# bayesian-optimization/BayesianOptimization

Measured on AMD Instinct MI355X. Metric: acquisition candidates/sec (suggest step: GP fit at fixed theta + posterior + acquisition + arg-best), higher is better.
Workload: dtype f64

## Files before the change

### bayesianoptimization_amd/csrc/posterior_kernel_v2.hip

```cpp
#include <type_traits>

#include "gpbo_internal.h"
#include "fit_bodies.h"
#include "i8_digits.h"
#include "posterior_tile.h"

namespace gpbo {

typedef double d4 __attribute__((ext_vector_type(4)));

constexpr int V2_CANDS = 64;
constexpr int V2_STRIDE = 64;

struct PostArgs2 {
  const double* Wp;
  const double* Xs;
  const double* alpha;
  const double* Xcs;
  double* part;
  double* mu_part;
  PostGrid g;
  const double* Kst;
  int64_t ldk;
  int64_t m0;
// ... 138 lines not shown

  __syncthreads();
  {
    double kv0[E];
    gen_compute(0, kv0, 1.0);
    gen_store(kv0, 0);
  }
  double2 aA[2], aB[2];
  loadA(0, aA);
  __syncthreads();

  const int last_stage = n_stages - 1;
  const int last_pair = (int)pairs - 1;
  auto stage = [&](int st, auto mode) {
    constexpr int MODE = decltype(mode)::value;
    const int buf = st & 1;
    double kv[E];
    if constexpr (MODE > 0) loadA(min(KP * st + 1, last_pair), aB);
    gen_compute(min(st + 1, last_stage), kv, st < last_stage ? 1.0 : 0.0);
    if constexpr (GEN == 2) __builtin_amdgcn_sched_barrier(0);
    if constexpr (MODE > 0) {
#pragma unroll
      for (int pp = 0; pp < KP; ++pp) {
        if (pp & 1) mma_pair(buf, pp, aB, mode);
        else mma_pair(buf, pp, aA, mode);
        if (pp + 1 < KP || (pp & 1) == 0) {
          if (pp & 1) loadA(min(KP * st + pp + 2, last_pair), aB);
          else loadA(min(KP * st + pp + 2, last_pair), aA);
        }
      }
    }
    gen_store(kv, buf ^ 1);
    __syncthreads();
  };
  const int sA = min(last_stage, (rowA0 + 15) / BK);
  const int sB = min(last_stage, (rowB0 + 15) / BK);
  int s = 0;
  for (; s <= sA; ++s) stage(s, both_t{});
  for (; s <= sB; ++s) stage(s, later_t{});
  for (; s <= last_stage; ++s) stage(s, std::integral_constant<int, 0>{});

  static_assert(2 * WAVES * V2_CANDS <= 2 * BK * V2_STRIDE, "the epilogue's exchange area aliases the stage tiles");
  double* red = Ks;
  double* mured = Ks + WAVES * V2_CANDS;
#pragma unroll
  for (int jt = 0; jt < 4; ++jt) {
    double v = 0.0;
#pragma unroll
    for (int rr = 0; rr < 4; ++rr) v = fma(acc[0][jt][rr], acc[0][jt][rr], v);
    if (!activeA) v = 0.0;
    double vb = 0.0;
#pragma unroll
    for (int rr = 0; rr < 4; ++rr) vb = fma(acc[1][jt][rr], acc[1][jt][rr], vb);
    if (activeB) v += vb;
    v += __shfl_xor(v, 16);
    v += __shfl_xor(v, 32);
    if (lane < 16) red[wave * V2_CANDS + jt * 16 + lane] = v;
  }
  mured[wave * V2_CANDS + lane] = mu_acc;
  __syncthreads();
  if (tid < V2_CANDS) {
    double v = 0.0;
#pragma unroll
    for (int w = 0; w < WAVES; ++w) v += red[w * V2_CANDS + tid];
    const int64_t m = p.m0 + (int64_t)ct * V2_CANDS + tid;
    if (GEN != 2 && p.fuse_ends) {
      double u = 0.0;
#pragma unroll
      for (int w = 0; w < WAVES; ++w) u += mured[w * V2_CANDS + tid];
      if (m < p.ends.M)
        posterior_finalize_elem(0.0 + v, 0.0 + u, p.ends.y_mean, p.ends.y_std, p.ends.amplitude, p.ends.white, p.ends.mu + m, p.ends.sd + m, p.ends.negvar);
      return;
    }
    p.part[(int64_t)r * p.g.Mp + m] = v;
    if (GEN != 2 && last) {
      double u = 0.0;
#pragma unroll
      for (int w = 0; w < WAVES; ++w) u += mured[w * V2_CANDS + tid];
      p.mu_part[m] = u;
    }
  }
}

constexpr int GEN_CH = 64;
template <PostPath SLAB> struct slab_value { using type = double; };
template <> struct slab_value<PostPath::SlabF32> { using type = float; };
template <int DP, int KERNEL, PostPath SLAB>
__global__ __launch_bounds__(256) void kstar_gen_kernel(const double* __restrict__ Xs, const double* __restrict__ alpha,
                                                        const double* __restrict__ Xcs, void* __restrict__ slab,
                                                        int64_t ldk, int NP, double* __restrict__ mu_part,
                                                        int64_t Mp, int64_t m0) {
  static_assert(SLAB == PostPath::SlabF64 || SLAB == PostPath::SlabF32 || SLAB == PostPath::SlabI8, "a slab path");
  __shared__ __attribute__((aligned(16))) double xs[GEN_CH * DP];
  __shared__ double al[GEN_CH];
  const int64_t ml = (int64_t)blockIdx.x * 256 + threadIdx.x;
  const bool live = ml < ldk;
  const int k0 = blockIdx.y * POST_ROWS, k1 = min(NP, k0 + POST_ROWS);
  double xc[DP];
  {
    const double* xcp = Xcs + (m0 + (live ? ml : 0)) * DP;
#pragma unroll
    for (int t = 0; t < DP; t += 2) {
      const double2 v = *reinterpret_cast<const double2*>(xcp + t);
      xc[t] = v.x;
      xc[t + 1] = v.y;
    }
  }
  double mu = 0.0;
  auto pair = [&](int kk, double& ka, double& kb) {
    const double* xr = xs + kk * DP;
    double d2a = 0.0, d2b = 0.0;
#pragma unroll
    for (int t = 0; t < DP; ++t) {
      const double da = xc[t] - xr[t], db = xc[t] - xr[DP + t];
      d2a = fma(da, da, d2a);
      d2b = fma(db, db, d2b);
    }
    ka = gpbo_kernel_value<KERNEL>(d2a);
    kb = gpbo_kernel_value<KERNEL>(d2b);
  };
  auto mean = [&](int kk, double ka, double kb) {
    mu = fma(ka, al[kk], mu);
    mu = fma(kb, al[kk + 1], mu);
  };
  for (int kc = k0; kc < k1; kc += GEN_CH) {
    __syncthreads();
    {
      const double2* src = reinterpret_cast<const double2*>(Xs + (int64_t)kc * DP);
      double2* dst = reinterpret_cast<double2*>(xs);
      for (int e = threadIdx.x; e < GEN_CH * DP / 2; e += 256) dst[e] = src[e];
      if (threadIdx.x < GEN_CH) al[threadIdx.x] = alpha[kc + threadIdx.x];
    }
    __syncthreads();
    if (!live) continue;
    if constexpr (SLAB == PostPath::SlabI8) {
      constexpr int S = I8_S;
      uint4* Kd = static_cast<uint4*>(slab);
      const int64_t cb = i8_kd_block(ml >> 4, NP);
#pragma unroll 1
      for (int kg = 0; kg < GEN_CH; kg += 16) {
        uint32_t w[S][4] = {};
#pragma unroll
        for (int kk = kg; kk < kg + 16; kk += 2) {
          double ka, kb;
          pair(kk, ka, kb);
          mean(kk, ka, kb);
          const int64_t qa = i8_quantize<S>(ka), qb = i8_quantize<S>(kb);
          const int j = kk - kg;
#pragma unroll
          for (int t = 0; t < S; ++t) {
            w[t][j >> 2] |= (uint32_t)((qa >> (8 * (S - 1 - t))) & 255) << (8 * (j & 3));
            w[t][j >> 2] |= (uint32_t)((qb >> (8 * (S - 1 - t))) & 255) << (8 * ((j + 1) & 3));
          }
        }
        const int k = kc + kg;
        uint4* dst = Kd + i8_frag_index<S>(cb, k, 0, (int)(ml & 15));
#pragma unroll
        for (int t = 0; t < S; ++t) {
          const uint32_t x = t ? 0x80808080u : 0u;
          dst[t * 64] = make_uint4(w[t][0] ^ x, w[t][1] ^ x, w[t][2] ^ x, w[t][3] ^ x);
        }
      }
    } else {
      using T = typename slab_value<SLAB>::type;
      T* Kst = static_cast<T*>(slab);
#pragma unroll 2
      for (int kk = 0; kk < GEN_CH; kk += 2) {
        double ka, kb;
        pair(kk, ka, kb);
        const int k = kc + kk;
        Kst[(int64_t)k * ldk + ml] = (T)ka;
        Kst[(int64_t)(k + 1) * ldk + ml] = (T)kb;
        mean(kk, ka, kb);
      }
    }
  }
  if (live) mu_part[(int64_t)blockIdx.y * Mp + m0 + ml] = mu;
}

template <PostPath SLAB>
static int launch_gen(gpbo_ctx* ctx, Model& m, void* slab, int64_t ldk, int64_t Mp, int64_t m0, int nchunks) {
  return with_dp_kernel(ctx, m.DP, m.kernel, [&](auto dp, auto k) {
    kstar_gen_kernel<decltype(dp)::value, decltype(k)::value, SLAB><<<dim3((unsigned)((ldk + 255) / 256), (unsigned)nchunks), dim3(256), 0,
                                                                      ctx->stream>>>(m.Xs, m.alpha, ctx->Xcs, slab, ldk, (int)m.NP,
                                                                                     ctx->mu_part, Mp, m0);
    GPBO_HIP(ctx, hipGetLastError());
    return GPBO_OK;
  });
}

int launch_kstar_slab(gpbo_ctx* ctx, Model& m, double* Kst, int64_t ldk, int64_t Mp, int64_t m0, int nchunks) {
  return launch_gen<PostPath::SlabF64>(ctx, m, Kst, ldk, Mp, m0, nchunks);
}
int launch_kstar_slab_f32(gpbo_ctx* ctx, Model& m, float* Kst, int64_t ldk, int64_t Mp, int64_t m0, int nchunks) {
  return launch_gen<PostPath::SlabF32>(ctx, m, Kst, ldk, Mp, m0, nchunks);
}
int launch_kstar_digits(gpbo_ctx* ctx, Model& m, void* Kd, int64_t ldk, int64_t Mp, int64_t m0, int nchunks) {
  return launch_gen<PostPath::SlabI8>(ctx, m, Kd, ldk, Mp, m0, nchunks);
}

static PostArgs2 post_args(gpbo_ctx* ctx, const Model& m, int64_t Mp, int nchunks, int64_t ncands) {
  PostArgs2 a;
  a.Wp = m.Wp; a.Xs = m.Xs; a.alpha = m.alpha; a.Xcs = ctx->Xcs; a.part = ctx->part; a.mu_part = ctx->mu_part;
  a.g = {(int)m.NP, Mp, nchunks, (int)(ncands / V2_CANDS)};
  a.Kst = nullptr; a.ldk = 0; a.m0 = 0;
  return a;
}

int launch_slab_gemm_f64(gpbo_ctx* ctx, Model& m, const double* slab, int64_t ldk, int64_t m0, int64_t Mp, int part_chunks) {
  PostArgs2 a = post_args(ctx, m, Mp, part_chunks, ldk);
  a.Kst = slab; a.ldk = ldk; a.m0 = m0;
  const size_t lds = (size_t)(2 * 32 * V2_STRIDE) * sizeof(double);
  posterior_kernel_v2<4, 0, 2, 32><<<dim3((unsigned)a.g.blocks()), dim3(512), lds, ctx->stream>>>(a);
  GPBO_HIP(ctx, hipGetLastError());
  return GPBO_OK;
}

int launch_posterior_fused(gpbo_ctx* ctx, Model& m, int64_t Mp, const PostPlan& plan, const PostEnds& ends) {
  if (plan.fuse_ends && plan.part_chunks != 1) GPBO_FAIL(ctx, GPBO_ERR_STATE, "posterior: fused ends need one row chunk");
  PostArgs2 a = post_args(ctx, m, Mp, plan.part_chunks, Mp);
  const int64_t nblocks = a.g.blocks();
  if (nblocks > 0x7fffffffLL) GPBO_FAIL(ctx, GPBO_ERR_UNSUPPORTED, "posterior: grid too large; shard the candidates");
  if (plan.fuse_ends) { a.fuse_ends = 1; a.ends = ends; }
  const bool wide = plan.path == PostPath::Fused512;
  return with_dp_kernel(ctx, m.DP, m.kernel, [&](auto dp, auto k) {
    constexpr int DP = decltype(dp)::value, KERNEL = decltype(k)::value;
    if (wide) {
      const size_t lds = (size_t)(2 * 32 * V2_STRIDE + DP * V2_CANDS) * sizeof(double);
      posterior_kernel_v2<DP, KERNEL, 1, 32, 16><<<dim3((unsigned)nblocks), dim3(1024), lds, ctx->stream>>>(a);
    } else {
      const size_t lds = (size_t)(2 * POST_BK * V2_STRIDE + DP * V2_CANDS) * sizeof(double);
      posterior_kernel_v2<DP, KERNEL, 1><<<dim3((unsigned)nblocks), dim3(512), lds, ctx->stream>>>(a);
    }
    GPBO_HIP(ctx, hipGetLastError());
    return GPBO_OK;
  });
}

}

#ifdef GPBO_DEBUG
using namespace gpbo;

int gpbo_debug_i8_kstar_digits(gpbo_ctx* ctx, int64_t NP, int64_t m0, int64_t ldk, void* Kd_out, double* kst_out, double* mu_part_out) {
  if (!ctx) return GPBO_ERR_INVALID;
  Model& m = ctx->models[0];
  if (!m.fitted || ctx->pending_info[0]) GPBO_FAIL(ctx, GPBO_ERR_STATE, "debug_i8_kstar_digits: model slot 0 has not been fitted");
  if (ctx->M < 1) GPBO_FAIL(ctx, GPBO_ERR_STATE, "debug_i8_kstar_digits: no candidates resident (call gpbo_set_candidates)");
  if (ctx->d_c != m.d) GPBO_FAIL(ctx, GPBO_ERR_INVALID, "debug_i8_kstar_digits: candidate dimension differs from the fitted model");
  const int64_t Mp = round_up(ctx->M, POST_CANDS);
  if (!Kd_out || !kst_out || !mu_part_out || m0 < 0 || ldk < 64 || m0 % 64 || ldk % 64 || m0 + ldk > Mp)
    GPBO_FAIL(ctx, GPBO_ERR_INVALID, "debug_i8_kstar_digits: bad arguments (m0, ldk multiples of 64 inside the padded candidate set)");
  if (m.NP > I8_NP_MAX || m.NP % 64) GPBO_FAIL(ctx, GPBO_ERR_UNSUPPORTED, "debug_i8_kstar_digits: the int8 GEMM serves NP <= 16384");
  if (NP != m.NP)
    GPBO_FAIL(ctx, GPBO_ERR_INVALID, "debug_i8_kstar_digits: NP is not the padded size of the model in slot 0");
  GPBO_HIP(ctx, hipSetDevice(ctx->device));
// ... 29 lines not shown
```

### bayesianoptimization_amd/csrc/posterior_plan.h

```cpp
#pragma once

#include <cstdint>

namespace gpbo {

constexpr int POST_ROWS = 256;
constexpr int POST_ROWS_WIDE = 512;
constexpr int POST_CANDS = 128;
constexpr int I8_ROWS = 128;
constexpr int64_t I8_NP_MIN = 2048;
constexpr int I8_NP_MAX = 16384;
constexpr int I8_S = 7;

enum class PostPath {
  Small,
  Fused256,
  Fused512,
  SlabF64,
  SlabI8,
  SlabF32,
};

struct PostPlan {
  PostPath path;
  bool fuse_ends;
  int part_chunks;
  int mu_chunks;
};

inline bool f32_use_mfma32(int64_t NP) { return NP >= POST_ROWS_WIDE; }

inline bool posterior_i8_serves(int64_t NP) { return NP >= I8_NP_MIN && NP <= I8_NP_MAX; }

struct SlabSpec {
  int64_t bytes_per_cand;
  int64_t offset_cap;
  bool narrow_ok;
};
inline SlabSpec slab_spec(PostPath path, int64_t NP) {
  switch (path) {
    case PostPath::SlabF64: return {8 * NP, (int64_t)80 * 1000 * 1000, false};
    case PostPath::SlabF32: return {4 * NP, (int64_t)160 * 1000 * 1000, false};
    case PostPath::SlabI8: return {I8_S * NP, INT64_MAX, true};
    default: return {0, 0, false};
  }
}
inline int64_t slab_doubles(int64_t ms, int64_t bytes_per_cand) { return (ms * bytes_per_cand + 7) / 8; }

constexpr int64_t I8_SLAB_BYTES = 256 * 1000 * 1000;
inline int64_t i8_slab_width(int64_t NP, int64_t bytes_per_cand, int64_t granted, int64_t compute_units) {
  const int64_t chunks = (NP + POST_ROWS - 1) / POST_ROWS;
  const int64_t kmax = I8_SLAB_BYTES / bytes_per_cand / 256;
  int64_t width = I8_SLAB_BYTES / bytes_per_cand / 128 * 128;
  int64_t best_wgs = 0, best_cap = 1;
  for (int64_t k = kmax; k >= 1 && 2 * k > kmax; --k) {
    const int64_t wgs = k * chunks, cap = (wgs + compute_units - 1) / compute_units * compute_units;
    if (wgs * best_cap > best_wgs * cap) { best_wgs = wgs; best_cap = cap; width = 256 * k; }
  }
  if (granted < width) width = granted;
  return width < 128 ? 128 : width;
}

inline PostPlan plan_posterior(int64_t NP, int64_t M, bool f32, int64_t gemv_limit, int force_kernel = 0, bool no_small = false,
                               bool no_fuse_ends = false) {
  const int nchunks = (int)((NP + POST_ROWS - 1) / POST_ROWS);
  const int64_t Mp = (M + POST_CANDS - 1) / POST_CANDS * POST_CANDS;
  if (M <= gemv_limit && !no_small) return {PostPath::Small, false, 0, 0};
  if (f32)
    return {PostPath::SlabF32, false, f32_use_mfma32(NP) ? (int)((NP + POST_ROWS_WIDE - 1) / POST_ROWS_WIDE) : nchunks, nchunks};
  PostPath path;
  if (nchunks <= 1) path = PostPath::Fused256;
  else if (nchunks == 2) {
    if (Mp < 8192) path = PostPath::Fused256;
    else if (Mp < 9216) path = PostPath::SlabF64;
    else if (Mp <= 16384) path = PostPath::Fused512;
    else if (Mp < 32768) path = PostPath::Fused256;
    else path = NP >= 384 ? PostPath::Fused512 : PostPath::SlabF64;
  } else path = posterior_i8_serves(NP) ? PostPath::SlabI8 : PostPath::SlabF64;
  switch (force_kernel) {
    case 2: path = PostPath::Fused256; break;
    case 3: path = PostPath::SlabF64; break;
    case 4: if (NP <= 1024) path = PostPath::Fused512; break;
    case 8: if (NP > 512 && NP <= I8_NP_MAX) path = PostPath::SlabI8; break;
  }
  PostPlan p{path, false, nchunks, nchunks};
  if (path == PostPath::Fused256 || path == PostPath::Fused512) {
    if (path == PostPath::Fused512) p.part_chunks = (int)((NP + POST_ROWS_WIDE - 1) / POST_ROWS_WIDE);
    p.mu_chunks = 1;
    p.fuse_ends = p.part_chunks == 1 && !no_fuse_ends;
  } else if (path == PostPath::SlabI8) {
    p.part_chunks = (int)((NP + I8_ROWS - 1) / I8_ROWS);
  }
  return p;
}

}
```

### bayesianoptimization_amd/csrc/i8_digits.h

```cpp
#pragma once

#include <cmath>
#include <cstdint>

#include "posterior_plan.h"

#if defined(__HIPCC__)
#define GPBO_HD __host__ __device__
#else
#define GPBO_HD
#endif

namespace gpbo {

static_assert((int64_t)I8_S * 128 * 128 * I8_NP_MAX < ((int64_t)1 << 31), "int32 level sums overflow at I8_NP_MAX");

template <int S>
GPBO_HD constexpr int64_t i8_offset() {
  int64_t o = 0;
  for (int t = 1; t < S; ++t) o = o * 256 + 128;
  return o;
}

GPBO_HD inline int64_t i8_round(double x) {
#if defined(__HIP_DEVICE_COMPILE__)
  return __double2ll_rn(x);
#else
  return (int64_t)std::nearbyint(x);
#endif
}

template <int S>
GPBO_HD inline int64_t i8_quantize(double x) {
  return i8_round(std::ldexp(x, 8 * S - 2)) + i8_offset<S>();
}

template <int S>
GPBO_HD inline uint32_t i8_digit_byte(int64_t Qo, int t) {
  return (uint32_t)((Qo >> (8 * (S - 1 - t))) & 255) ^ (t ? 128u : 0u);
}

GPBO_HD inline int i8_row_exponent(double maxabs) {
  int e = 0;
  (void)std::frexp(maxabs, &e);
  return maxabs > 0.0 ? e : 0;
}

template <int S>
GPBO_HD constexpr int64_t i8_frag_index(int64_t first_step, int64_t k, int plane, int item) {
  return ((first_step + (k >> 6)) * S + plane) * 64 + ((k >> 4) & 3) * 16 + item;
}
GPBO_HD constexpr int64_t i8_kd_block(int64_t cb, int64_t NP) { return cb * (NP / 64); }
GPBO_HD constexpr int64_t i8_wd_block(int64_t b) {
  const int64_t q = b >> 2, r = b & 3;
  return b + 2 * q * (q - 1) + r * q;
}

template <int S>
GPBO_HD inline double i8_combine(const int32_t* acc) {
  static_assert(S >= 5 && S <= 7, "groups of S - 4, 2 and 2 levels");
  double h = 0.0;
  for (int l = 0; l < S - 4; ++l) h = h * 256.0 + (double)acc[l];
  h *= 4294967296.0;
  const double m = (double)acc[S - 4] * 16777216.0 + (double)acc[S - 3] * 65536.0;
  const double lo = (double)acc[S - 2] * 256.0 + (double)acc[S - 1];
  const double s = h + m;
  const double bb = s - h;
  const double e = (h - (s - bb)) + (m - bb);
  return s + (e + lo);
}

template <int S>
GPBO_HD constexpr int i8_scale_exp(int e) {
  return e - 2 * (8 * S - 2) + 8 * (S - 1);
}

}
```

### bayesianoptimization_amd/csrc/posterior_i8.hip

```cpp
#include <algorithm>

#include "gpbo_internal.h"
#include "i8_digits.h"
#include "posterior_tile.h"

namespace gpbo {

typedef int v4i __attribute__((ext_vector_type(4)));

constexpr int I8_CANDS = 64;

__global__ __launch_bounds__(256) void wd_row_scale_kernel(const double* __restrict__ W, int* __restrict__ wexp,
                                                           double* __restrict__ wscale, int64_t N, int64_t NP) {
  const int64_t row = (int64_t)blockIdx.x * 4 + (threadIdx.x >> 6);
  const int lane = threadIdx.x & 63;
  if (row >= NP) return;
  double mx = 0.0;
  if (row < N)
    for (int64_t j = lane; j <= row; j += 64) mx = fmax(mx, fabs(W[row * NP + j]));
#pragma unroll
  for (int o = 32; o > 0; o >>= 1) mx = fmax(mx, __shfl_xor(mx, o));
  if (lane == 0) {
    const int e = i8_row_exponent(mx);
    wexp[row] = e;
    wscale[row] = ldexp(1.0, i8_scale_exp<I8_S>(e));
  }
}

__global__ __launch_bounds__(256) void wd_pack_kernel(const double* __restrict__ W, const int* __restrict__ wexp,
                                                      uint4* __restrict__ Wd, int64_t N, int64_t NP) {
  const int b = blockIdx.y;
  const int t = blockIdx.x * 256 + threadIdx.x;
  const int ks = t >> 6, lane = t & 63;
  if (ks > b / 4) return;
  const int64_t row = (int64_t)b * 16 + (lane & 15);
  const int64_t c0 = (int64_t)ks * 64 + (lane >> 4) * 16;
  const int e = wexp[row];
  uint32_t w[I8_S][4] = {};
#pragma unroll
  for (int j = 0; j < 16; ++j) {
    const int64_t col = c0 + j;
    const double x = (row < N && col < N && col <= row) ? W[row * NP + col] : 0.0;
    const int64_t q = i8_quantize<I8_S>(ldexp(x, -e));
#pragma unroll
    for (int s = 0; s < I8_S; ++s) w[s][j >> 2] |= i8_digit_byte<I8_S>(q, s) << (8 * (j & 3));
  }
  uint4* dst = Wd + i8_frag_index<I8_S>(i8_wd_block(b), c0, 0, lane & 15);
#pragma unroll
  for (int s = 0; s < I8_S; ++s) dst[s * 64] = make_uint4(w[s][0], w[s][1], w[s][2], w[s][3]);
}

static int pack_wd(gpbo_ctx* ctx, Model& m) {
  const int64_t nb = m.NP / 16;
  int rc;
  if ((rc = ensure(ctx, &m.Wd, &m.cap_Wd, i8_wd_block(nb) * I8_S * 64))) return rc;
  if ((rc = ensure(ctx, &m.wscale, &m.cap_wscale, 2 * m.NP))) return rc;
  int* wexp = reinterpret_cast<int*>(m.wscale + m.NP);
  wd_row_scale_kernel<<<dim3((unsigned)((m.NP + 3) / 4)), dim3(256), 0, ctx->stream>>>(m.W, wexp, m.wscale, m.N, m.NP);
  GPBO_HIP(ctx, hipGetLastError());
  wd_pack_kernel<<<dim3((unsigned)((m.NP + 255) / 256), (unsigned)nb), dim3(256), 0, ctx->stream>>>(m.W, wexp, m.Wd, m.N, m.NP);
  GPBO_HIP(ctx, hipGetLastError());
  m.wd_valid = true;
  return GPBO_OK;
}

struct I8Args {
  const uint4* Wd;
  const double* wscale;
  const uint4* Kd;
  double* part;
  PostGrid g;
  int64_t m0;
};

template <int S>
__global__ __launch_bounds__(256, 1) void posterior_i8_kernel(I8Args p) {
  const int tid = threadIdx.x;
  const int wave = __builtin_amdgcn_readfirstlane(tid >> 6);
  const int lane = tid & 63;
  int r, ct;
  p.g.map(blockIdx.x, r, ct);
  const int nks = p.g.NP / 64;
  const int rb = r * (I8_ROWS / 32) + wave;
  const bool active = rb < p.g.NP / 32;

  __shared__ double red[4][I8_CANDS];
  double ss[4] = {0.0, 0.0, 0.0, 0.0};
  if (active) {
    v4i acc[2][4][S];
#pragma unroll
    for (int a = 0; a < 2; ++a)
#pragma unroll
      for (int j = 0; j < 4; ++j)
#pragma unroll
        for (int l = 0; l < S; ++l) acc[a][j][l] = v4i{};
    const int n = rb / 2 + 1;
    const uint4* wa = p.Wd + i8_wd_block(2 * rb) * S * 64;
    const uint4* kb0 = p.Kd + i8_kd_block(4 * ct, p.g.NP) * S * 64;
    const __amdgpu_buffer_rsrc_t rsA = __builtin_amdgcn_make_buffer_rsrc(const_cast<uint4*>(wa), 0, 0x7fffffff, BUF_FLAGS);
    const __amdgpu_buffer_rsrc_t rsB = __builtin_amdgcn_make_buffer_rsrc(const_cast<uint4*>(kb0), 0, 0x7fffffff, BUF_FLAGS);
    const unsigned voff = (unsigned)lane * 16u;
    const unsigned sofA = (unsigned)n * S * 1024u, sofB = (unsigned)nks * S * 1024u;
    v4i a[2][S], b[4][S];
    auto load_a = [&](int ks, int i) {
      const unsigned o = (unsigned)ks * S * 1024u + i * sofA;
#pragma unroll
      for (int s = 0; s < S; ++s)
        a[i][s] = __builtin_bit_cast(v4i, __builtin_amdgcn_raw_buffer_load_b128(rsA, voff, o + s * 1024u, 0));
    };
    auto load_b = [&](int ks, int j0) {
      const unsigned o = (unsigned)ks * S * 1024u;
#pragma unroll
      for (int s = 0; s < S; ++s)
#pragma unroll
        for (int j = j0; j < j0 + 2; ++j)
          b[j][s] = __builtin_bit_cast(v4i, __builtin_amdgcn_raw_buffer_load_b128(rsB, voff, o + j * sofB + s * 1024u, 0));
    };
    auto mma = [&](int i, int j0) {
#pragma unroll
      for (int s = 0; s < S; ++s)
#pragma unroll
        for (int t = 0; t + s < S; ++t)
#pragma unroll
          for (int j = j0; j < j0 + 2; ++j)
            acc[i][j][s + t] = __builtin_amdgcn_mfma_i32_16x16x64_i8(a[i][s], b[j][t], acc[i][j][s + t], 0, 0, 0);
    };
    load_a(0, 0);
    load_b(0, 0);
    __builtin_amdgcn_sched_barrier(0);
    load_a(0, 1);
    __builtin_amdgcn_sched_barrier(0);
    load_b(0, 2);
#pragma unroll 1
    for (int ks = 0; ks < n; ++ks) {
      const int nx = min(ks + 1, n - 1);
      __builtin_amdgcn_sched_barrier(0);
      mma(0, 0);
      __builtin_amdgcn_sched_barrier(0);
      mma(1, 0);
      __builtin_amdgcn_sched_barrier(0);
      load_b(nx, 0);
      __builtin_amdgcn_sched_barrier(0);
      mma(0, 2);
      __builtin_amdgcn_sched_barrier(0);
      load_a(nx, 0);
      __builtin_amdgcn_sched_barrier(0);
      mma(1, 2);
      __builtin_amdgcn_sched_barrier(0);
      load_a(nx, 1);
      load_b(nx, 2);
    }

#pragma unroll
    for (int j = 0; j < 4; ++j) {
      double s = 0.0;
#pragma unroll
      for (int a = 0; a < 2; ++a) {
        double v[4];
#pragma unroll
        for (int i = 0; i < 4; ++i) {
          const int row = rb * 32 + 16 * a + 4 * (lane >> 4) + i;
          int32_t lv[S];
#pragma unroll
          for (int l = 0; l < S; ++l) lv[l] = acc[a][j][l][i];
          v[i] = i8_combine<S>(lv) * p.wscale[row];
          __builtin_amdgcn_sched_barrier(0);
        }
#pragma unroll
        for (int i = 0; i < 4; ++i) s = fma(v[i], v[i], s);
        s = __shfl_xor(s, 32);
#pragma unroll
        for (int i = 0; i < 4; ++i) s = fma(v[i], v[i], s);
        if (a == 0) s = __shfl_xor(s, 32);
      }
      ss[j] = s;
    }
  }
#pragma unroll
  for (int j = 0; j < 4; ++j) {
    const double o = __shfl_xor(ss[j], 16);
    if ((lane >> 4) == 2) red[wave][j * 16 + (lane & 15)] = ss[j] + o;
  }
  __syncthreads();
  if (tid < I8_CANDS) {
    const double v = ((red[0][tid] + red[1][tid]) + red[2][tid]) + red[3][tid];
    p.part[(int64_t)r * p.g.Mp + p.m0 + (int64_t)ct * I8_CANDS + tid] = v;
  }
}

static int launch_i8_gemm(gpbo_ctx* ctx, const uint4* Wd, const double* wscale, const uint4* Kd, double* part, int64_t NP, int64_t Mp,
                          int nchunks, int64_t ldk, int64_t m0) {
  I8Args a;
  a.Wd = Wd; a.wscale = wscale; a.Kd = Kd; a.part = part;
  a.g = {(int)NP, Mp, nchunks, (int)(ldk / I8_CANDS)};
  a.m0 = m0;
  posterior_i8_kernel<I8_S><<<dim3((unsigned)a.g.blocks()), dim3(256), 0, ctx->stream>>>(a);
  GPBO_HIP(ctx, hipGetLastError());
  return GPBO_OK;
}

int launch_slab_gemm_i8(gpbo_ctx* ctx, Model& m, const void* slab, int64_t ldk, int64_t m0, int64_t Mp, int part_chunks) {
  return launch_i8_gemm(ctx, m.Wd, m.wscale, static_cast<const uint4*>(slab), ctx->part, m.NP, Mp, part_chunks, ldk, m0);
}

int prepare_posterior_i8(gpbo_ctx* ctx, Model& m) {
  if (m.NP > I8_NP_MAX || m.NP % 64) GPBO_FAIL(ctx, GPBO_ERR_UNSUPPORTED, "posterior: the int8 GEMM serves NP <= 16384");
  int rc;
  if (!m.wd_valid && (rc = pack_wd(ctx, m))) return rc;
  if (!ctx->compute_units) GPBO_HIP(ctx, hipDeviceGetAttribute(&ctx->compute_units, hipDeviceAttributeMultiprocessorCount, ctx->device));
  return GPBO_OK;
}

}

#ifdef GPBO_DEBUG
using namespace gpbo;

static bool i8_debug_np_ok(int64_t NP) { return NP >= 64 && NP <= I8_NP_MAX && NP % 64 == 0; }

int gpbo_debug_i8_pack_w(gpbo_ctx* ctx, const double* W, int64_t N, int64_t NP, void* Wd_out, int* wexp_out, double* wscale_out) {
  if (!ctx) return GPBO_ERR_INVALID;
  if (!W || !Wd_out || !wexp_out || !wscale_out || !i8_debug_np_ok(NP) || N < 1 || N > NP)
    GPBO_FAIL(ctx, GPBO_ERR_INVALID, "debug_i8_pack_w: bad arguments (NP a multiple of 64 in [64, 16384], 1 <= N <= NP)");
  GPBO_HIP(ctx, hipSetDevice(ctx->device));
  Model m;
  m.N = N; m.NP = NP;
  auto done = [&](int code) {
    if (m.W) (void)hipFree(m.W);
    if (m.Wd) (void)hipFree(m.Wd);
    if (m.wscale) (void)hipFree(m.wscale);
    return code;
  };
  const size_t sq = (size_t)NP * NP * sizeof(double);
  if (hipMalloc((void**)&m.W, sq) != hipSuccess) return done(GPBO_ERR_HIP);
  if (hipMemcpy(m.W, W, sq, hipMemcpyHostToDevice) != hipSuccess) return done(GPBO_ERR_HIP);
  int rc = pack_wd(ctx, m);
  if (rc) return done(rc);
  if (hipStreamSynchronize(ctx->stream) != hipSuccess) return done(GPBO_ERR_HIP);
  const size_t wd_bytes = (size_t)i8_wd_block(NP / 16) * I8_S * 64 * sizeof(uint4);
  if (hipMemcpy(Wd_out, m.Wd, wd_bytes, hipMemcpyDeviceToHost) != hipSuccess) return done(GPBO_ERR_HIP);
  if (hipMemcpy(wscale_out, m.wscale, (size_t)NP * sizeof(double), hipMemcpyDeviceToHost) != hipSuccess) return done(GPBO_ERR_HIP);
  if (hipMemcpy(wexp_out, m.wscale + NP, (size_t)NP * sizeof(int), hipMemcpyDeviceToHost) != hipSuccess) return done(GPBO_ERR_HIP);
  return done(GPBO_OK);
}

int gpbo_debug_i8_gemm(gpbo_ctx* ctx, const void* Wd, const double* wscale, const void* Kd, int64_t NP, int64_t M, double* part_out) {
  if (!ctx) return GPBO_ERR_INVALID;
  if (!Wd || !wscale || !Kd || !part_out || !i8_debug_np_ok(NP) || M < I8_CANDS || M % I8_CANDS || M > (1 << 20))
    GPBO_FAIL(ctx, GPBO_ERR_INVALID, "debug_i8_gemm: bad arguments (NP a multiple of 64 in [64, 16384], M a multiple of 64)");
  GPBO_HIP(ctx, hipSetDevice(ctx->device));
  const int nchunks = (int)((NP + I8_ROWS - 1) / I8_ROWS);
  const size_t wd_bytes = (size_t)i8_wd_block(NP / 16) * I8_S * 64 * sizeof(uint4);
  const size_t kd_bytes = (size_t)M * NP * I8_S;
  const size_t part_bytes = (size_t)nchunks * M * sizeof(double);
  uint4 *dW = nullptr, *dK = nullptr;
  double *dS = nullptr, *dP = nullptr;
  auto done = [&](int code) {
    if (dW) (void)hipFree(dW);
    if (dK) (void)hipFree(dK);
    if (dS) (void)hipFree(dS);
    if (dP) (void)hipFree(dP);
    return code;
  };
  if (hipMalloc((void**)&dW, wd_bytes) != hipSuccess || hipMalloc((void**)&dK, kd_bytes) != hipSuccess ||
      hipMalloc((void**)&dS, (size_t)NP * sizeof(double)) != hipSuccess || hipMalloc((void**)&dP, part_bytes) != hipSuccess)
    return done(GPBO_ERR_HIP);
  if (hipMemcpy(dW, Wd, wd_bytes, hipMemcpyHostToDevice) != hipSuccess || hipMemcpy(dK, Kd, kd_bytes, hipMemcpyHostToDevice) != hipSuccess ||
      hipMemcpy(dS, wscale, (size_t)NP * sizeof(double), hipMemcpyHostToDevice) != hipSuccess ||
      hipMemset(dP, 0xff, part_bytes) != hipSuccess)
    return done(GPBO_ERR_HIP);
  const int rc = launch_i8_gemm(ctx, dW, dS, dK, dP, NP, M, nchunks, M, 0);
  if (rc) return done(rc);
  if (hipStreamSynchronize(ctx->stream) != hipSuccess) return done(GPBO_ERR_HIP);
  if (hipMemcpy(part_out, dP, part_bytes, hipMemcpyDeviceToHost) != hipSuccess) return done(GPBO_ERR_HIP);
  return done(GPBO_OK);
}
#endif
```

Before: 6.108 million.

## Software-pipeline LDS reads in K* slab generator with register ring and larger staging

The slab generation kernel now stages up to 32KB of training points per sync (up to POST_ROWS points instead of a fixed 64). Distance computation is split into 4-dimension pieces, prefetched from LDS into a register ring one or more pieces ahead, with sched_barrier and asm pins keeping loads overlapped with FMAs. Alpha for the next pair is also prefetched. This is meant to hide LDS latency and reduce syncthreads count, at the cost of more registers and occupancy risk.

```diff
diff --git a/bayesianoptimization_amd/csrc/posterior_kernel_v2.hip b/bayesianoptimization_amd/csrc/posterior_kernel_v2.hip
--- a/bayesianoptimization_amd/csrc/posterior_kernel_v2.hip
+++ b/bayesianoptimization_amd/csrc/posterior_kernel_v2.hip
@@ -244,7 +244,9 @@
   }
 }
 
-constexpr int GEN_CH = 64;
+#define GEN_PIN(a, b) asm volatile("" : "+v"(a), "+v"(b) : : "memory")
+constexpr int GEN_PIECE = 4;
+constexpr int gen_ring_slots(int DP) { return DP >= 64 ? 2 : DP / GEN_PIECE < 4 ? DP / GEN_PIECE : 4; }
 template <PostPath SLAB> struct slab_value { using type = double; };
 template <> struct slab_value<PostPath::SlabF32> { using type = float; };
 template <int DP, int KERNEL, PostPath SLAB>
@@ -253,8 +255,13 @@
                                                         int64_t ldk, int NP, double* __restrict__ mu_part,
                                                         int64_t Mp, int64_t m0) {
   static_assert(SLAB == PostPath::SlabF64 || SLAB == PostPath::SlabF32 || SLAB == PostPath::SlabI8, "a slab path");
-  __shared__ __attribute__((aligned(16))) double xs[GEN_CH * DP];
-  __shared__ double al[GEN_CH];
+  constexpr int PTS = gen_stage_points(DP);
+  constexpr int NPIECE = DP / GEN_PIECE;
+  constexpr int RING = gen_ring_slots(DP);
+  static_assert(DP % GEN_PIECE == 0 && NPIECE % RING == 0, "a piece's ring slot is its index modulo the ring, the same in every pair");
+  static_assert(PTS >= 64 && PTS % 64 == 0 && POST_ROWS % PTS == 0, "whole groups of 64 points, a whole number of stagings per chunk");
+  __shared__ __attribute__((aligned(16))) double xs[PTS * DP];
+  __shared__ __attribute__((aligned(16))) double al[PTS];
   const int64_t ml = (int64_t)blockIdx.x * 256 + threadIdx.x;
   const bool live = ml < ldk;
   const int k0 = blockIdx.y * POST_ROWS, k1 = min(NP, k0 + POST_ROWS);
@@ -269,44 +276,73 @@
     }
   }
   double mu = 0.0;
-  auto pair = [&](int kk, double& ka, double& kb) {
-    const double* xr = xs + kk * DP;
+  double ring[RING][2 * GEN_PIECE];
+  double2 ac, an;
+  auto fetch = [&](int j, int kk) {
+    const double2* pa = reinterpret_cast<const double2*>(xs + kk * DP + GEN_PIECE * j);
+#pragma unroll
+    for (int h = 0; h < 2; ++h) {
+      const double2 u = pa[h * (DP / 2)], v = pa[h * (DP / 2) + 1];
+      double* r = ring[j % RING] + GEN_PIECE * h;
+      r[0] = u.x; r[1] = u.y; r[2] = v.x; r[3] = v.y;
+    }
+  };
+  auto prime = [&]() {
+#pragma unroll
+    for (int j = 0; j < RING; ++j) fetch(j, 0);
+    an = *reinterpret_cast<const double2*>(al);
+  };
+  auto pair = [&](int kk, int kn, double& ka, double& kb) {
+    ac = an;
     double d2a = 0.0, d2b = 0.0;
 #pragma unroll
-    for (int t = 0; t < DP; ++t) {
-      const double da = xc[t] - xr[t], db = xc[t] - xr[DP + t];
-      d2a = fma(da, da, d2a);
-      d2b = fma(db, db, d2b);
+    for (int j = 0; j < NPIECE; ++j) {
+      const double* r = ring[j % RING];
+#pragma unroll
+      for (int t = 0; t < GEN_PIECE; ++t) {
+        const double da = xc[GEN_PIECE * j + t] - r[t], db = xc[GEN_PIECE * j + t] - r[GEN_PIECE + t];
+        d2a = fma(da, da, d2a);
+        d2b = fma(db, db, d2b);
+      }
+      GEN_PIN(d2a, d2b);
+      __builtin_amdgcn_sched_barrier(0);
+      if (j + RING < NPIECE) fetch(j + RING, kk);
+      else fetch(j + RING - NPIECE, kn);
+      if (j == NPIECE - 1) an = *reinterpret_cast<const double2*>(al + kn);
+      __builtin_amdgcn_sched_barrier(0);
     }
     ka = gpbo_kernel_value<KERNEL>(d2a);
     kb = gpbo_kernel_value<KERNEL>(d2b);
   };
-  auto mean = [&](int kk, double ka, double kb) {
-    mu = fma(ka, al[kk], mu);
-    mu = fma(kb, al[kk + 1], mu);
-  };
-  for (int kc = k0; kc < k1; kc += GEN_CH) {
-    __syncthreads();
+  auto mean = [&](double ka, double kb) {
+    mu = fma(ka, ac.x, mu);
+    mu = fma(kb, ac.y, mu);
+  };
+  for (int kc = k0; kc < k1; kc += PTS) {
+    const int np = min(PTS, k1 - kc);
+    if (kc > k0) __syncthreads();
     {
       const double2* src = reinterpret_cast<const double2*>(Xs + (int64_t)kc * DP);
       double2* dst = reinterpret_cast<double2*>(xs);
-      for (int e = threadIdx.x; e < GEN_CH * DP / 2; e += 256) dst[e] = src[e];
-      if (threadIdx.x < GEN_CH) al[threadIdx.x] = alpha[kc + threadIdx.x];
+      for (int e = threadIdx.x; e < np * (DP / 2); e += 256) dst[e] = src[e];
+      if (threadIdx.x < np) al[threadIdx.x] = alpha[kc + threadIdx.x];
     }
     __syncthreads();
     if (!live) continue;
+    const int klast = np - 2;
+    prime();
     if constexpr (SLAB == PostPath::SlabI8) {
       constexpr int S = I8_S;
       uint4* Kd = static_cast<uint4*>(slab);
       const int64_t cb = i8_kd_block(ml >> 4, NP);
 #pragma unroll 1
-      for (int kg = 0; kg < GEN_CH; kg += 16) {
+      for (int kg = 0; kg < np; kg += 16) {
         uint32_t w[S][4] = {};
 #pragma unroll
         for (int kk = kg; kk < kg + 16; kk += 2) {
           double ka, kb;
-          pair(kk, ka, kb);
-          mean(kk, ka, kb);
+          pair(kk, min(kk + 2, klast), ka, kb);
+          mean(ka, kb);
           const int64_t qa = i8_quantize<S>(ka), qb = i8_quantize<S>(kb);
           const int j = kk - kg;
 #pragma unroll
@@ -326,14 +362,17 @@
     } else {
       using T = typename slab_value<SLAB>::type;
       T* Kst = static_cast<T*>(slab);
-#pragma unroll 2
-      for (int kk = 0; kk < GEN_CH; kk += 2) {
-        double ka, kb;
-        pair(kk, ka, kb);
-        const int k = kc + kk;
-        Kst[(int64_t)k * ldk + ml] = (T)ka;
-        Kst[(int64_t)(k + 1) * ldk + ml] = (T)kb;
-        mean(kk, ka, kb);
+#pragma unroll 1
+      for (int kq = 0; kq < np; kq += 4) {
+#pragma unroll
+        for (int kk = kq; kk < kq + 4; kk += 2) {
+          double ka, kb;
+          pair(kk, min(kk + 2, klast), ka, kb);
+          const int k = kc + kk;
+          Kst[(int64_t)k * ldk + ml] = (T)ka;
+          Kst[(int64_t)(k + 1) * ldk + ml] = (T)kb;
+          mean(ka, kb);
+        }
       }
     }
   }
diff --git a/bayesianoptimization_amd/csrc/posterior_plan.h b/bayesianoptimization_amd/csrc/posterior_plan.h
--- a/bayesianoptimization_amd/csrc/posterior_plan.h
+++ b/bayesianoptimization_amd/csrc/posterior_plan.h
@@ -47,6 +47,12 @@
 }
 inline int64_t slab_doubles(int64_t ms, int64_t bytes_per_cand) { return (ms * bytes_per_cand + 7) / 8; }
 
+constexpr int GEN_STAGE_BYTES = 32 * 1024;
+constexpr int gen_stage_points(int DP) {
+  const int fit = GEN_STAGE_BYTES / (8 * DP) / 64 * 64;
+  return fit < POST_ROWS ? fit : POST_ROWS;
+}
+
 constexpr int64_t I8_SLAB_BYTES = 256 * 1000 * 1000;
 inline int64_t i8_slab_width(int64_t NP, int64_t bytes_per_cand, int64_t granted, int64_t compute_units) {
   const int64_t chunks = (NP + POST_ROWS - 1) / POST_ROWS;
```

After: 6.141 million (median of 6 runs). No clear change (+0.5%).

## Walk paired triangular row chunks per block to balance int8 posterior GEMM

Applied to the files above, without the earlier changes.

Each block now processes a set of up to four row chunks, pairing a long chunk from the bottom of the triangular W with a short one from the top. This balances the work per block, and keeping the B (candidate kernel) fragments resident across the walk lets them be reused. Loads for the next row block are prefetched in the final k-step, so consecutive chunks pipeline without a drain. Row scales are staged in shared memory instead of being read from global memory in the epilogue. The cost is more shared memory, fewer and longer blocks that may reduce parallelism, and more complex indexing.

```diff
diff --git a/bayesianoptimization_amd/csrc/i8_digits.h b/bayesianoptimization_amd/csrc/i8_digits.h
--- a/bayesianoptimization_amd/csrc/i8_digits.h
+++ b/bayesianoptimization_amd/csrc/i8_digits.h
@@ -56,6 +56,36 @@
   return b + 2 * q * (q - 1) + r * q;
 }
 
+constexpr int I8_WALK = 4;
+
+template <int WALK>
+GPBO_HD constexpr int i8_walk_sets(int nchunks) {
+  static_assert(WALK == 2 || WALK == 4, "a set is one or two pairs of chunks");
+  const int npairs = nchunks / 2, per = WALK / 2;
+  return (npairs + per - 1) / per + (nchunks & 1);
+}
+template <int WALK>
+GPBO_HD constexpr int i8_walk_len(int nchunks, int set) {
+  const int left = nchunks / 2 - set * (WALK / 2);
+  return left <= 0 ? 1 : 2 * (left < WALK / 2 ? left : WALK / 2);
+}
+template <int WALK>
+GPBO_HD constexpr int i8_walk_chunk(int nchunks, int set, int pos) {
+  const int p0 = set * (WALK / 2), len = i8_walk_len<WALK>(nchunks, set);
+  if (len == 1) return nchunks / 2;
+  return pos < len / 2 ? nchunks - 1 - (p0 + pos) : p0 + (len - 1 - pos);
+}
+GPBO_HD constexpr int i8_walk_row_block(int pos, int wave) { return (pos & 1) ? 3 - wave : wave; }
+GPBO_HD constexpr void i8_walk_block(int bid, int n_ctiles, int& set, int& ct) {
+  set = bid / n_ctiles;
+  ct = bid - set * n_ctiles;
+}
+template <int WALK>
+GPBO_HD constexpr int64_t i8_walk_blocks(int nchunks, int n_ctiles) {
+  return (int64_t)i8_walk_sets<WALK>(nchunks) * n_ctiles;
+}
+GPBO_HD constexpr int i8_row_block_steps(int rb) { return rb / 2 + 1; }
+
 template <int S>
 GPBO_HD inline double i8_combine(const int32_t* acc) {
   static_assert(S >= 5 && S <= 7, "groups of S - 4, 2 and 2 levels");
diff --git a/bayesianoptimization_amd/csrc/posterior_i8.hip b/bayesianoptimization_amd/csrc/posterior_i8.hip
--- a/bayesianoptimization_amd/csrc/posterior_i8.hip
+++ b/bayesianoptimization_amd/csrc/posterior_i8.hip
@@ -78,113 +78,159 @@
   const int tid = threadIdx.x;
   const int wave = __builtin_amdgcn_readfirstlane(tid >> 6);
   const int lane = tid & 63;
-  int r, ct;
-  p.g.map(blockIdx.x, r, ct);
+  int set, ct;
+  i8_walk_block(blockIdx.x, p.g.n_ctiles, set, ct);
+  const int nchunks = p.g.nchunks;
+  const int len = i8_walk_len<I8_WALK>(nchunks, set);
   const int nks = p.g.NP / 64;
-  const int rb = r * (I8_ROWS / 32) + wave;
-  const bool active = rb < p.g.NP / 32;
-
-  __shared__ double red[4][I8_CANDS];
-  double ss[4] = {0.0, 0.0, 0.0, 0.0};
-  if (active) {
-    v4i acc[2][4][S];
-#pragma unroll
-    for (int a = 0; a < 2; ++a)
-#pragma unroll
-      for (int j = 0; j < 4; ++j)
-#pragma unroll
-        for (int l = 0; l < S; ++l) acc[a][j][l] = v4i{};
-    const int n = rb / 2 + 1;
-    const uint4* wa = p.Wd + i8_wd_block(2 * rb) * S * 64;
-    const uint4* kb0 = p.Kd + i8_kd_block(4 * ct, p.g.NP) * S * 64;
-    const __amdgpu_buffer_rsrc_t rsA = __builtin_amdgcn_make_buffer_rsrc(const_cast<uint4*>(wa), 0, 0x7fffffff, BUF_FLAGS);
-    const __amdgpu_buffer_rsrc_t rsB = __builtin_amdgcn_make_buffer_rsrc(const_cast<uint4*>(kb0), 0, 0x7fffffff, BUF_FLAGS);
-    const unsigned voff = (unsigned)lane * 16u;
-    const unsigned sofA = (unsigned)n * S * 1024u, sofB = (unsigned)nks * S * 1024u;
-    v4i a[2][S], b[4][S];
-    auto load_a = [&](int ks, int i) {
-      const unsigned o = (unsigned)ks * S * 1024u + i * sofA;
-#pragma unroll
-      for (int s = 0; s < S; ++s)
-        a[i][s] = __builtin_bit_cast(v4i, __builtin_amdgcn_raw_buffer_load_b128(rsA, voff, o + s * 1024u, 0));
-    };
-    auto load_b = [&](int ks, int j0) {
-      const unsigned o = (unsigned)ks * S * 1024u;
-#pragma unroll
-      for (int s = 0; s < S; ++s)
-#pragma unroll
-        for (int j = j0; j < j0 + 2; ++j)
-          b[j][s] = __builtin_bit_cast(v4i, __builtin_amdgcn_raw_buffer_load_b128(rsB, voff, o + j * sofB + s * 1024u, 0));
-    };
-    auto mma = [&](int i, int j0) {
-#pragma unroll
-      for (int s = 0; s < S; ++s)
-#pragma unroll
-        for (int t = 0; t + s < S; ++t)
-#pragma unroll
-          for (int j = j0; j < j0 + 2; ++j)
-            acc[i][j][s + t] = __builtin_amdgcn_mfma_i32_16x16x64_i8(a[i][s], b[j][t], acc[i][j][s + t], 0, 0, 0);
-    };
-    load_a(0, 0);
+  const int nrb = p.g.NP / 32;
+  auto row_block = [&](int pos) {
+    return i8_walk_chunk<I8_WALK>(nchunks, set, pos) * (I8_ROWS / 32) + i8_walk_row_block(pos, wave);
+  };
+
+  __shared__ double wsl[4][I8_WALK][32];
+  __shared__ double red[I8_WALK][4][I8_CANDS];
+  const uint4* kb0 = p.Kd + i8_kd_block(4 * ct, p.g.NP) * S * 64;
+  const __amdgpu_buffer_rsrc_t rsA = __builtin_amdgcn_make_buffer_rsrc(const_cast<uint4*>(p.Wd), 0, 0x7fffffff, BUF_FLAGS);
+  const __amdgpu_buffer_rsrc_t rsB = __builtin_amdgcn_make_buffer_rsrc(const_cast<uint4*>(kb0), 0, 0x7fffffff, BUF_FLAGS);
+  const unsigned voff = (unsigned)lane * 16u;
+  const unsigned sofB = (unsigned)nks * S * 1024u;
+  v4i a[2][S], b[4][S];
+  auto load_a = [&](unsigned oa, unsigned sa, int i) {
+    const unsigned o = oa + i * sa;
+#pragma unroll
+    for (int s = 0; s < S; ++s)
+      a[i][s] = __builtin_bit_cast(v4i, __builtin_amdgcn_raw_buffer_load_b128(rsA, voff, o + s * 1024u, 0));
+  };
+  auto load_b = [&](unsigned ob, int j0) {
+#pragma unroll
+    for (int s = 0; s < S; ++s)
+#pragma unroll
+      for (int j = j0; j < j0 + 2; ++j)
+        b[j][s] = __builtin_bit_cast(v4i, __builtin_amdgcn_raw_buffer_load_b128(rsB, voff, ob + j * sofB + s * 1024u, 0));
+  };
+  auto first_loads = [&](int rb) {
+    const unsigned oa = (unsigned)i8_wd_block(2 * rb) * S * 1024u, sa = (unsigned)i8_row_block_steps(rb) * S * 1024u;
+    load_a(oa, sa, 0);
     load_b(0, 0);
     __builtin_amdgcn_sched_barrier(0);
-    load_a(0, 1);
+    load_a(oa, sa, 1);
     __builtin_amdgcn_sched_barrier(0);
     load_b(0, 2);
+  };
+
+  auto put_red = [&](int pos, const double (&ss)[4]) {
+    const int rbk = i8_walk_row_block(pos, wave);
+#pragma unroll
+    for (int j = 0; j < 4; ++j) {
+      const double o = __shfl_xor(ss[j], 16);
+      if ((lane >> 4) == 2) red[pos][rbk][j * 16 + (lane & 15)] = ss[j] + o;
+    }
+  };
+  double wv[I8_WALK / 2];
+#pragma unroll
+  for (int h = 0; h < I8_WALK / 2; ++h) {
+    const int ps = 2 * h + (lane >> 5);
+    const int r = (ps < len ? row_block(ps) : nrb) * 32 + (lane & 31);
+    wv[h] = r < p.g.NP ? p.wscale[r] : 0.0;
+  }
+  int pos = 0;
+  while (pos < len && row_block(pos) >= nrb) {
+    const double zero[4] = {0.0, 0.0, 0.0, 0.0};
+    put_red(pos++, zero);
+  }
+  if (pos < len) first_loads(row_block(pos));
+#pragma unroll
+  for (int h = 0; h < I8_WALK / 2; ++h) wsl[wave][2 * h + (lane >> 5)][lane & 31] = wv[h];
+  __builtin_amdgcn_wave_barrier();
 #pragma unroll 1
-    for (int ks = 0; ks < n; ++ks) {
-      const int nx = min(ks + 1, n - 1);
-      __builtin_amdgcn_sched_barrier(0);
-      mma(0, 0);
-      __builtin_amdgcn_sched_barrier(0);
-      mma(1, 0);
-      __builtin_amdgcn_sched_barrier(0);
-      load_b(nx, 0);
-      __builtin_amdgcn_sched_barrier(0);
-      mma(0, 2);
-      __builtin_amdgcn_sched_barrier(0);
-      load_a(nx, 0);
-      __builtin_amdgcn_sched_barrier(0);
-      mma(1, 2);
-      __builtin_amdgcn_sched_barrier(0);
-      load_a(nx, 1);
-      load_b(nx, 2);
+  for (; pos < len; ++pos) {
+    const int rb = row_block(pos);
+    const bool more = pos + 1 < len;
+    const int rb_next = more ? row_block(pos + 1) : rb;
+    double ss[4];
+    {
+      v4i acc[2][4][S];
+#pragma unroll
+      for (int i = 0; i < 2; ++i)
+#pragma unroll
+        for (int j = 0; j < 4; ++j)
+#pragma unroll
+          for (int l = 0; l < S; ++l) acc[i][j][l] = v4i{};
+      auto mma = [&](int i, int j0) {
+#pragma unroll
+        for (int s = 0; s < S; ++s)
+#pragma unroll
+          for (int t = 0; t + s < S; ++t)
+#pragma unroll
+            for (int j = j0; j < j0 + 2; ++j)
+              acc[i][j][s + t] = __builtin_amdgcn_mfma_i32_16x16x64_i8(a[i][s], b[j][t], acc[i][j][s + t], 0, 0, 0);
+      };
+      const int n = i8_row_block_steps(rb);
+      const unsigned oa0 = (unsigned)i8_wd_block(2 * rb) * S * 1024u, sa0 = (unsigned)n * S * 1024u;
+      const unsigned oa_end = more ? (unsigned)i8_wd_block(2 * rb_next) * S * 1024u : oa0 + (unsigned)(n - 1) * S * 1024u;
+      const unsigned sa_end = more ? (unsigned)i8_row_block_steps(rb_next) * S * 1024u : sa0;
+      const unsigned ob_end = more ? 0u : (unsigned)(n - 1) * S * 1024u;
+#pragma unroll 1
+      for (int ks = 1; ks <= n; ++ks) {
+        const bool last = ks == n;
+        const unsigned oa = last ? oa_end : oa0 + (unsigned)ks * S * 1024u, sa = last ? sa_end : sa0;
+        const unsigned ob = last ? ob_end : (unsigned)ks * S * 1024u;
+        __builtin_amdgcn_sched_barrier(0);
+        mma(0, 0);
+        __builtin_amdgcn_sched_barrier(0);
+        mma(1, 0);
+        __builtin_amdgcn_sched_barrier(0);
+        load_b(ob, 0);
+        __builtin_amdgcn_sched_barrier(0);
+        mma(0, 2);
+        __builtin_amdgcn_sched_barrier(0);
+        load_a(oa, sa, 0);
+        __builtin_amdgcn_sched_barrier(0);
+        mma(1, 2);
+        __builtin_amdgcn_sched_barrier(0);
+        load_a(oa, sa, 1);
+        load_b(ob, 2);
+      }
+
+      double wsc[2][4];
+#pragma unroll
+      for (int i = 0; i < 2; ++i)
+#pragma unroll
+        for (int q = 0; q < 4; ++q) wsc[i][q] = wsl[wave][pos][16 * i + 4 * (lane >> 4) + q];
+#pragma unroll
+      for (int j = 0; j < 4; ++j) {
+        double s = 0.0;
+#pragma unroll
+        for (int i = 0; i < 2; ++i) {
+          double v[4];
+#pragma unroll
+          for (int l = 0; l < S; ++l) asm volatile("" : "+a"(acc[i][j][l]));
+#pragma unroll
+          for (int q = 0; q < 4; ++q) {
+            int32_t lv[S];
+#pragma unroll
+            for (int l = 0; l < S; ++l) lv[l] = acc[i][j][l][q];
+            v[q] = i8_combine<S>(lv) * wsc[i][q];
+            __builtin_amdgcn_sched_barrier(0);
+          }
+#pragma unroll
+          for (int q = 0; q < 4; ++q) s = fma(v[q], v[q], s);
+          s = __shfl_xor(s, 32);
+#pragma unroll
+          for (int q = 0; q < 4; ++q) s = fma(v[q], v[q], s);
+          if (i == 0) s = __shfl_xor(s, 32);
+        }
+        ss[j] = s;
+      }
     }
-
-#pragma unroll
-    for (int j = 0; j < 4; ++j) {
-      double s = 0.0;
-#pragma unroll
-      for (int a = 0; a < 2; ++a) {
-        double v[4];
-#pragma unroll
-        for (int i = 0; i < 4; ++i) {
-          const int row = rb * 32 + 16 * a + 4 * (lane >> 4) + i;
-          int32_t lv[S];
-#pragma unroll
-          for (int l = 0; l < S; ++l) lv[l] = acc[a][j][l][i];
-          v[i] = i8_combine<S>(lv) * p.wscale[row];
-          __builtin_amdgcn_sched_barrier(0);
-        }
-#pragma unroll
-        for (int i = 0; i < 4; ++i) s = fma(v[i], v[i], s);
-        s = __shfl_xor(s, 32);
-#pragma unroll
-        for (int i = 0; i < 4; ++i) s = fma(v[i], v[i], s);
-        if (a == 0) s = __shfl_xor(s, 32);
-      }
-      ss[j] = s;
-    }
-  }
-#pragma unroll
-  for (int j = 0; j < 4; ++j) {
-    const double o = __shfl_xor(ss[j], 16);
-    if ((lane >> 4) == 2) red[wave][j * 16 + (lane & 15)] = ss[j] + o;
+    put_red(pos, ss);
   }
   __syncthreads();
-  if (tid < I8_CANDS) {
-    const double v = ((red[0][tid] + red[1][tid]) + red[2][tid]) + red[3][tid];
-    p.part[(int64_t)r * p.g.Mp + p.m0 + (int64_t)ct * I8_CANDS + tid] = v;
+  if (tid < len * I8_CANDS) {
+    const int pos = tid >> 6, c = tid & 63;
+    const double v = ((red[pos][0][c] + red[pos][1][c]) + red[pos][2][c]) + red[pos][3][c];
+    p.part[(int64_t)i8_walk_chunk<I8_WALK>(nchunks, set, pos) * p.g.Mp + p.m0 + (int64_t)ct * I8_CANDS + c] = v;
   }
 }
 
@@ -194,7 +240,7 @@
   a.Wd = Wd; a.wscale = wscale; a.Kd = Kd; a.part = part;
   a.g = {(int)NP, Mp, nchunks, (int)(ldk / I8_CANDS)};
   a.m0 = m0;
-  posterior_i8_kernel<I8_S><<<dim3((unsigned)a.g.blocks()), dim3(256), 0, ctx->stream>>>(a);
+  posterior_i8_kernel<I8_S><<<dim3((unsigned)i8_walk_blocks<I8_WALK>(nchunks, a.g.n_ctiles)), dim3(256), 0, ctx->stream>>>(a);
   GPBO_HIP(ctx, hipGetLastError());
   return GPBO_OK;
 }
```

Result: no change. 5.772 million before, 5.768 million after (-0.1%).

## Stage larger K* gen chunks in LDS and software-pipeline training-point reads

Applied to the files above, without the earlier changes.

The K* generation kernel now sizes its LDS staging chunk from the dimension count, up to 64KB, instead of a fixed 64 points. This means fewer workgroup barriers per row range, and launch bounds request two workgroups per CU. The distance loop is split into dimension units. Reads of the next unit, or of the next point pair, are issued from LDS before the current FMAs, with sched barriers forcing the overlap. This hides LDS latency at the cost of more registers and more complex scheduling, and the partial-chunk handling now clamps to the remaining rows.

```diff
diff --git a/bayesianoptimization_amd/csrc/posterior_kernel_v2.hip b/bayesianoptimization_amd/csrc/posterior_kernel_v2.hip
--- a/bayesianoptimization_amd/csrc/posterior_kernel_v2.hip
+++ b/bayesianoptimization_amd/csrc/posterior_kernel_v2.hip
@@ -244,17 +244,29 @@
   }
 }
 
-constexpr int GEN_CH = 64;
+constexpr int GEN_LDS_BYTES = 64 * 1024;
+constexpr int gen_stage_points(int DP) {
+  const int fit = GEN_LDS_BYTES / ((DP + 1) * 8) / 64 * 64;
+  return fit < POST_ROWS ? fit : POST_ROWS;
+}
+constexpr int gen_unit_dims(int DP) { return DP <= 16 ? DP : DP == 32 ? 8 : 4; }
+static_assert(gen_stage_points(4) == 256 && gen_stage_points(16) == 256 && gen_stage_points(32) == 192 && gen_stage_points(64) == 64,
+              "stage sizes");
 template <PostPath SLAB> struct slab_value { using type = double; };
 template <> struct slab_value<PostPath::SlabF32> { using type = float; };
 template <int DP, int KERNEL, PostPath SLAB>
-__global__ __launch_bounds__(256) void kstar_gen_kernel(const double* __restrict__ Xs, const double* __restrict__ alpha,
-                                                        const double* __restrict__ Xcs, void* __restrict__ slab,
-                                                        int64_t ldk, int NP, double* __restrict__ mu_part,
-                                                        int64_t Mp, int64_t m0) {
+__global__ __launch_bounds__(256, 2) void kstar_gen_kernel(const double* __restrict__ Xs, const double* __restrict__ alpha,
+                                                           const double* __restrict__ Xcs, void* __restrict__ slab,
+                                                           int64_t ldk, int NP, double* __restrict__ mu_part,
+                                                           int64_t Mp, int64_t m0) {
   static_assert(SLAB == PostPath::SlabF64 || SLAB == PostPath::SlabF32 || SLAB == PostPath::SlabI8, "a slab path");
+  constexpr int GEN_CH = gen_stage_points(DP);
+  constexpr int TB = gen_unit_dims(DP), NU = DP / TB;
+  constexpr int TA = TB + 1 > 15 ? 12 : TB;
+  static_assert(GEN_CH >= 64 && GEN_CH % 64 == 0 && 2 * GEN_CH * (DP + 1) * 8 <= 160 * 1024, "stages of whole 64-steps, two workgroups per CU");
+  static_assert(DP % TB == 0 && TB % 2 == 0, "units of whole 16-byte reads");
   __shared__ __attribute__((aligned(16))) double xs[GEN_CH * DP];
-  __shared__ double al[GEN_CH];
+  __shared__ __attribute__((aligned(16))) double al[GEN_CH];
   const int64_t ml = (int64_t)blockIdx.x * 256 + threadIdx.x;
   const bool live = ml < ldk;
   const int k0 = blockIdx.y * POST_ROWS, k1 = min(NP, k0 + POST_ROWS);
@@ -269,44 +281,83 @@
     }
   }
   double mu = 0.0;
-  auto pair = [&](int kk, double& ka, double& kb) {
-    const double* xr = xs + kk * DP;
+  double cx[2][TB], nx[2][TB];
+  double ca[2], na[2];
+  auto fetch = [&](int kk, int u, int t0, int t1, double (&x)[2][TB]) {
+    const double* xr = xs + kk * DP + u * TB;
+#pragma unroll
+    for (int t = t0; t < t1; ++t) {
+      x[0][t] = xr[t];
+      x[1][t] = xr[DP + t];
+    }
+  };
+  auto fetch_first = [&]() {
+    fetch(0, 0, 0, TB, cx);
+    ca[0] = al[0];
+    ca[1] = al[1];
+  };
+  auto pair = [&](int kk, int kn, double& ka, double& kb) {
     double d2a = 0.0, d2b = 0.0;
 #pragma unroll
-    for (int t = 0; t < DP; ++t) {
-      const double da = xc[t] - xr[t], db = xc[t] - xr[DP + t];
-      d2a = fma(da, da, d2a);
-      d2b = fma(db, db, d2b);
+    for (int u = 0; u < NU; ++u) {
+      const bool last = u + 1 == NU;
+      const int fk = last ? kn : kk, fu = last ? 0 : u + 1;
+      fetch(fk, fu, 0, TA, nx);
+      __builtin_amdgcn_sched_barrier(0);
+      asm volatile("" : "+v"(d2a), "+v"(d2b));
+#pragma unroll
+      for (int t = 0; t < TB; ++t) {
+        const double da = xc[u * TB + t] - cx[0][t], db = xc[u * TB + t] - cx[1][t];
+        d2a = fma(da, da, d2a);
+        d2b = fma(db, db, d2b);
+      }
+      asm volatile("" : "+v"(d2a), "+v"(d2b));
+      __builtin_amdgcn_sched_barrier(0);
+      fetch(fk, fu, TA, TB, nx);
+      if (last) {
+        na[0] = al[kn];
+        na[1] = al[kn + 1];
+      }
+      if (last || TA < TB) __builtin_amdgcn_sched_barrier(0);
+#pragma unroll
+      for (int t = 0; t < TB; ++t) {
+        cx[0][t] = nx[0][t];
+        cx[1][t] = nx[1][t];
+      }
     }
     ka = gpbo_kernel_value<KERNEL>(d2a);
     kb = gpbo_kernel_value<KERNEL>(d2b);
   };
-  auto mean = [&](int kk, double ka, double kb) {
-    mu = fma(ka, al[kk], mu);
-    mu = fma(kb, al[kk + 1], mu);
+  auto mean = [&](double ka, double kb) {
+    mu = fma(ka, ca[0], mu);
+    mu = fma(kb, ca[1], mu);
+    ca[0] = na[0];
+    ca[1] = na[1];
   };
   for (int kc = k0; kc < k1; kc += GEN_CH) {
+    const int n = min(GEN_CH, k1 - kc);
     __syncthreads();
     {
       const double2* src = reinterpret_cast<const double2*>(Xs + (int64_t)kc * DP);
       double2* dst = reinterpret_cast<double2*>(xs);
-      for (int e = threadIdx.x; e < GEN_CH * DP / 2; e += 256) dst[e] = src[e];
-      if (threadIdx.x < GEN_CH) al[threadIdx.x] = alpha[kc + threadIdx.x];
+      for (int e = threadIdx.x; e < n * DP / 2; e += 256) dst[e] = src[e];
+      if (threadIdx.x < n) al[threadIdx.x] = alpha[kc + threadIdx.x];
     }
     __syncthreads();
     if (!live) continue;
+    fetch_first();
     if constexpr (SLAB == PostPath::SlabI8) {
       constexpr int S = I8_S;
       uint4* Kd = static_cast<uint4*>(slab);
       const int64_t cb = i8_kd_block(ml >> 4, NP);
 #pragma unroll 1
-      for (int kg = 0; kg < GEN_CH; kg += 16) {
+      for (int kg = 0; kg < n; kg += 16) {
         uint32_t w[S][4] = {};
 #pragma unroll
         for (int kk = kg; kk < kg + 16; kk += 2) {
           double ka, kb;
-          pair(kk, ka, kb);
-          mean(kk, ka, kb);
+          pair(kk, min(kk + 2, n - 2), ka, kb);
+          mean(ka, kb);
           const int64_t qa = i8_quantize<S>(ka), qb = i8_quantize<S>(kb);
           const int j = kk - kg;
 #pragma unroll
@@ -326,14 +377,17 @@
     } else {
       using T = typename slab_value<SLAB>::type;
       T* Kst = static_cast<T*>(slab);
-#pragma unroll 2
-      for (int kk = 0; kk < GEN_CH; kk += 2) {
-        double ka, kb;
-        pair(kk, ka, kb);
-        const int k = kc + kk;
-        Kst[(int64_t)k * ldk + ml] = (T)ka;
-        Kst[(int64_t)(k + 1) * ldk + ml] = (T)kb;
-        mean(kk, ka, kb);
+#pragma unroll 1
+      for (int kq = 0; kq < n; kq += 4) {
+#pragma unroll
+        for (int kk = kq; kk < kq + 4; kk += 2) {
+          double ka, kb;
+          pair(kk, min(kk + 2, n - 2), ka, kb);
+          const int k = kc + kk;
+          Kst[(int64_t)k * ldk + ml] = (T)ka;
+          Kst[(int64_t)(k + 1) * ldk + ml] = (T)kb;
+          mean(ka, kb);
+        }
       }
     }
   }
```

Result: no change. 6.011 million before, 6.051 million after (median of 6 runs) (+0.7%).
